# anuragranj/cc

Hardware: AMD Instinct MI355X
Metric: train images/sec (832x256, 5-frame sample, 6-scale CC step) (higher is better)
Workload: dtype f32; 1 GPU; full CC: DispResNet6+PoseNetB6+MaskNet6+Back2Future, all losses; per_gpu_batch=4, global_batch=4, height=256, width=832, scales=6, frames=5, parallelism=dp1, hipgraph=True, trained_nets=all, rccl_ranks=1, dead_occlusion_decoders_elided=False, net_streams=2, pipeline=per_network, grad_chunks=False, deterministic=True

## Files before the change

cc_amd/build.py:

```python
import glob
import os
import subprocess
import sys
from concurrent.futures import ThreadPoolExecutor

HERE = os.path.dirname(os.path.abspath(__file__))
CSRC = os.path.join(HERE, "csrc")
OUT = os.path.join(HERE, "libccengine.so")
OBJ = os.path.join(HERE, "csrc", "_obj")
HIPCC = os.environ.get("HIPCC", "/opt/rocm/bin/hipcc")
FLAGS = ["--offload-arch=gfx950", "-O3", "-std=c++17", "-fPIC", "-ffp-contract=off",
         "-Wno-unused-result", "-I", os.path.join(os.path.dirname(HERE), "include")]


FILE_FLAGS = {"ssim.hip": ["-fno-slp-vectorize"]}


def sources():
    return sorted(glob.glob(os.path.join(CSRC, "*.hip")))


def _stale(target, deps):
    if not os.path.exists(target):
        return True
    t = os.path.getmtime(target)
    return any(os.path.getmtime(d) > t for d in deps)


def source_hash():
    import hashlib
    h = hashlib.sha1()
    files = sorted(glob.glob(os.path.join(CSRC, "*.hip")) + glob.glob(os.path.join(CSRC, "*.h")) +
                   glob.glob(os.path.join(os.path.dirname(HERE), "include", "*.h")))
    for f in files:
        h.update(os.path.basename(f).encode())
        h.update(open(f, "rb").read())
    return int(h.hexdigest()[:8], 16)


TOOLS_OUT = os.path.join(os.path.dirname(HERE), "tools", "_bin", "libccengine_tools.so")


def build_tools(verbose=False, force=False):
    return build(verbose, force, out=TOOLS_OUT, obj=os.path.join(CSRC, "_obj_tools"), extra=["-DCC_TOOLS"])


def build(verbose=False, force=False, out=None, obj=None, extra=()):
    OUT_, OBJ_ = out or OUT, obj or OBJ
# ... 42 lines not shown
```

cc_amd/config.py:

```python
align_corners = False

strict_nan_checks = False

deterministic = True

net_streams = True


grad_chunks = False

bias_table = False

loss_stream = True


class _Debug:
    no_slice_gy = False
    no_wgrad_defer = False
    no_sum_n = False
    no_wgrad_list = False
    no_wgrad_queue = False
    force_comm = False
    capture_mode = "thread_local"
    net_stream_priority = (0, 0, 0)
    chunk_inline = False
    pipe_extra = {}
    pipe_skip_tail = ()
    reduce_trace = None
    library_path = None


debug = _Debug()
```

cc_amd/csrc/corr.hip:

```cpp
#include "cc_common.h"
#include "../../include/ccengine.h"

namespace {

constexpr int R = 4, PATCH = 9, ND = 81;

__global__ __launch_bounds__(256) void k_corr_fwd(const float* __restrict__ f1, const float* __restrict__ f2,
                                                  float* __restrict__ out, const int* __restrict__ chan_of_disp, int C,
                                                  int H, int W, int out_cstride_total, int out_coffset) {
    const int HW = H * W;
    const int p = blockIdx.x * 256 + threadIdx.x;
    const int dy = blockIdx.y, b = blockIdx.z;
    if (p >= HW) return;
    const int y = p / W, x = p - y * W;
    const int yy = y + dy - R;
    float acc[PATCH];
#pragma unroll
    for (int j = 0; j < PATCH; j++) acc[j] = 0.f;
    if (yy >= 0 && yy < H) {
        const float* a = f1 + (size_t)b * C * HW + p;
        const float* bb = f2 + (size_t)b * C * HW + yy * W;
        for (int c = 0; c < C; c++) {
            const float av = a[(size_t)c * HW];
            const float* row = bb + (size_t)c * HW;
// ... 290 lines not shown
    out[((size_t)b * ND2 + d) * HW + p] = acc / (float)C;
}

__global__ __launch_bounds__(256) void k_corrp_bwd(const float* __restrict__ gout, const float* __restrict__ f1,
                                                   const float* __restrict__ f2, float* __restrict__ g1, float* __restrict__ g2,
                                                   int C, int H, int W, int P, int D) {
    const int HW = H * W, ND2 = P * P, r = (P - 1) / 2;
    const int p = blockIdx.x * 256 + threadIdx.x;
    const int c = blockIdx.y, b = blockIdx.z;
    if (p >= HW) return;
    const int y = p / W, x = p - y * W;
    const float* g = gout + (size_t)b * ND2 * HW;
    const float* s1 = f1 + ((size_t)b * C + c) * HW;
    const float* s2 = f2 + ((size_t)b * C + c) * HW;
    float a1 = 0.f, a2 = 0.f;
    for (int i = 0; i < P; i++) {
        const int dy = (i - r) * D;
        for (int j = 0; j < P; j++) {
            const int dx = (j - r) * D, d = i * P + j;
            const int yy = y + dy, xx = x + dx;
            if (yy >= 0 && yy < H && xx >= 0 && xx < W) a1 = fmaf(g[(size_t)d * HW + p], s2[yy * W + xx], a1);
            const int ys = y - dy, xs = x - dx;
            if (ys >= 0 && ys < H && xs >= 0 && xs < W) {
                const int q = ys * W + xs;
                a2 = fmaf(g[(size_t)d * HW + q], s1[q], a2);
            }
        }
    }
    const size_t o = ((size_t)b * C + c) * HW + p;
    if (g1) g1[o] = a1 / (float)C;
    if (g2) g2[o] = a2 / (float)C;
}

}

extern "C" {

int cc_corr9x9_fwd(const float* f1, const float* f2, float* out, const int* chan_of_disp_or_null, int B, int C, int H,
                   int W, int out_channels_total, int out_channel_offset, void* stream) {
    if (B <= 0 || C <= 0 || H <= 0 || W <= 0 || out_channel_offset + ND > out_channels_total) return CC_ERR_ARG;
    const bool v4 = (W % 4 == 0) && (((uintptr_t)f1 | (uintptr_t)f2 | (uintptr_t)out) % 16 == 0);
    if (v4)
        hipLaunchKernelGGL(k_corr_fwd4, dim3((H * (W / 4) + 255) / 256, PATCH, B), dim3(256), 0, (hipStream_t)stream, f1, f2, out,
                           chan_of_disp_or_null, C, H, W, out_channels_total, out_channel_offset);
    else if (H * W <= 4096)
        hipLaunchKernelGGL(k_corr_fwd_small, dim3((H * W * ND + 255) / 256, B), dim3(256), 0, (hipStream_t)stream, f1, f2, out,
                           chan_of_disp_or_null, C, H, W, out_channels_total, out_channel_offset);
    else
        hipLaunchKernelGGL(k_corr_fwd, dim3((H * W + 255) / 256, PATCH, B), dim3(256), 0, (hipStream_t)stream, f1, f2, out,
                           chan_of_disp_or_null, C, H, W, out_channels_total, out_channel_offset);
    CC_CHECK_LAUNCH();
    return CC_OK;
}

int cc_corr9x9_bwd(const float* gout, const float* f1, const float* f2, float* g1, float* g2_or_null,
                   const int* chan_of_disp_or_null, int B, int C, int H, int W, int g_channels_total,
                   int g_channel_offset, int accumulate_g1, void* stream) {
    if (B <= 0 || C <= 0 || H <= 0 || W <= 0 || g_channel_offset + ND > g_channels_total) return CC_ERR_ARG;
    hipStream_t s = (hipStream_t)stream;
    const bool v4 = (W % 4 == 0) &&
                    (((uintptr_t)gout | (uintptr_t)f1 | (uintptr_t)f2 | (uintptr_t)g1 | (uintptr_t)g2_or_null) % 16 == 0);
    if (v4) {
        dim3 g4((H * (W / 4) + 255) / 256, (C + 3) / 4, B);
        hipLaunchKernelGGL(k_corr_bwd_f1_4, g4, dim3(256), 0, s, gout, f2, g1, chan_of_disp_or_null, C, H, W, g_channels_total,
                           g_channel_offset, accumulate_g1);
        if (g2_or_null)
            hipLaunchKernelGGL(k_corr_bwd_f2_4, g4, dim3(256), 0, s, gout, f1, g2_or_null, chan_of_disp_or_null, C, H, W,
                               g_channels_total, g_channel_offset);
        CC_CHECK_LAUNCH();
        return CC_OK;
    }
    dim3 g((H * W + 255) / 256, C, B);
    hipLaunchKernelGGL(k_corr_bwd_f1, g, dim3(256), 0, s, gout, f2, g1, chan_of_disp_or_null, C, H, W, g_channels_total,
                       g_channel_offset, accumulate_g1);
    if (g2_or_null)
        hipLaunchKernelGGL(k_corr_bwd_f2, g, dim3(256), 0, s, gout, f1, g2_or_null, chan_of_disp_or_null, C, H, W,
                           g_channels_total, g_channel_offset);
    CC_CHECK_LAUNCH();
    return CC_OK;
}

int cc_corr_patch_fwd(const float* f1, const float* f2, float* out, int B, int C, int H, int W, int patch, int dilation,
                      void* stream) {
    if (B <= 0 || C <= 0 || H <= 0 || W <= 0 || patch < 1 || (patch & 1) == 0 || dilation < 1) return CC_ERR_ARG;
    const long n = (long)H * W * patch * patch;
    hipLaunchKernelGGL(k_corrp_fwd, dim3((unsigned)((n + 255) / 256), B), dim3(256), 0, (hipStream_t)stream, f1, f2, out, C, H, W,
                       patch, dilation);
    CC_CHECK_LAUNCH();
    return CC_OK;
}

int cc_corr_patch_bwd(const float* gout, const float* f1, const float* f2, float* g1_or_null, float* g2_or_null, int B, int C,
                      int H, int W, int patch, int dilation, void* stream) {
    if (B <= 0 || C <= 0 || H <= 0 || W <= 0 || patch < 1 || (patch & 1) == 0 || dilation < 1) return CC_ERR_ARG;
    hipLaunchKernelGGL(k_corrp_bwd, dim3((H * W + 255) / 256, C, B), dim3(256), 0, (hipStream_t)stream, gout, f1, f2, g1_or_null,
                       g2_or_null, C, H, W, patch, dilation);
    CC_CHECK_LAUNCH();
    return CC_OK;
}

}
```

cc_amd/models/back2future.py:

```python
import torch
import torch.nn as nn
import torch.nn.functional as F

from .. import config
from .. import nn as L
from .. import ops
from ..inverse_warp import feature_warp
from ..tape import run_network


def conv_feat_block(nIn, nOut):
    return nn.Sequential(L.Conv2d(nIn, nOut, 3, 2, 1, act="lrelu"), L.Act(),
                         L.Conv2d(nOut, nOut, 3, 1, 1, act="lrelu"), L.Act())


def conv_dec_block(nIn):
    chans = [nIn, 128, 128, 96, 64, 32]
    layers = []
    for a, b in zip(chans[:-1], chans[1:]):
        layers += [L.Conv2d(a, b, 3, 1, 1, act="lrelu"), L.Act()]
    layers.append(L.Conv2d(32, 2, 3, 1, 1))
    return nn.Sequential(*layers)


# ... 55 lines not shown
                out = tape.conv_group([xs[k] for k in idx], [convs[k].weight for k in idx], [convs[k].bias for k in idx], 1, 1, act)
                for k, y in zip(idx, out):
                    ys[k] = y
            xs = ys
        return xs

    def _body(self, tape, n0, n1, n2):
        ac = config.align_corners
        feats = {}
        xs = [n0, n2, n1]
        for lvl in range(1, 7):
            blocks = [getattr(self, "conv%d%s" % (lvl, s)) for s in "abc"]
            ys = tape.conv_group(xs, [b[0].weight for b in blocks], [b[0].bias for b in blocks], 2, 1, "lrelu")
            xs = tape.conv_group(ys, [b[2].weight for b in blocks], [b[2].bias for b in blocks], 1, 1, "lrelu")
            for s, x in zip("abc", xs):
                feats[(lvl, s)] = x
        flow_f, flow_b, up_f, up_b, occ_raw = {}, {}, {}, {}, {}
        bw, cw = feats[(6, "b")], feats[(6, "c")]
        inv_b, inv_c = ops._inv_perm(self.idx_fwd, n0.t.device), ops._inv_perm(self.idx_bwd, n0.t.device)
        for lvl in range(6, 1, -1):
            a = feats[(lvl, "a")]
            B, C, H, W = a.t.shape
            if lvl == 6:
                cb_o = tape.concat(B, [162, C], H, W, a.t) if not self.elide_occ else None
                corr = tape.corr_pair(a, bw, cw, inv_b, inv_c, out=cb_o.slot(0) if cb_o is not None else None)
                in_f = in_b = corr
                if cb_o is not None:
                    cb_o.put(0, corr)
                    cb_o.put(1, a)
                    in_o = cb_o.done()
            else:
                cb_f = tape.concat(B, [162, C, 2], H, W, a.t)
                cb_b = tape.concat(B, [162, C, 2], H, W, a.t)
                corr = tape.corr_pair(a, bw, cw, inv_b, inv_c, out=cb_f.slot(0))
                cb_f.put(0, corr)
                cb_f.put(1, a)
                cb_f.put(2, up_f[lvl + 1])
                cb_b.buf[:, :162 + C].copy_(cb_f.buf[:, :162 + C])
                cb_b.parts[0], cb_b.parts[1] = corr, a
                cb_b.put(2, up_b[lvl + 1])
                in_f, in_b = cb_f.done(), cb_b.done()
                in_o = in_f
            decs = [getattr(self, "decoder_fwd%d" % lvl), getattr(self, "decoder_bwd%d" % lvl)]
            ins = [in_f, in_b]
            if not self.elide_occ:
                decs.append(getattr(self, "decoder_occ%d" % lvl))
                ins.append(in_o)
            outs = self._decoders(tape, decs, ins)
            flow_f[lvl], flow_b[lvl] = outs[0], outs[1]
            up_f[lvl] = tape.upsample2x(flow_f[lvl])
            up_b[lvl] = tape.upsample2x(flow_b[lvl])
            if not self.elide_occ:
                occ_raw[lvl] = outs[2]
            if lvl > 2:
                s = self.WARP_SCALE[lvl]
                bw = tape.feature_warp(feats[(lvl - 1, "b")], up_f[lvl], s, ac)
                cw = tape.feature_warp(feats[(lvl - 1, "c")], up_f[lvl], -s, ac)
        ff = [tape.upsample2x(up_f[l], self.FULL_SCALE[l]) for l in range(2, 7)]
        fb = [tape.upsample2x(up_b[l], -self.FULL_SCALE[l]) for l in range(2, 7)]
        if self.training and self.nlevels == 6:
            ff += tape.torch_fn([up_f[6]], lambda t: (0.625 * t,))
            fb += tape.torch_fn([up_b[6]], lambda t: (-0.625 * t,))
        if not self.training:
            ff, fb = ff[:1], fb[:1]
        self._n_flow = len(ff)
        return ff + fb + [occ_raw[l] for l in sorted(occ_raw)]

    def forward(self, im_tar, im_refs):
        n = self.normalize([im_tar] + list(im_refs))
        outs = list(run_network(self._body, n, list(self.parameters())))
        k = self._n_flow
# ... 11 lines not shown
```

cc_amd/ops.py:

```python
import torch
import torch.nn.functional as F

from ._lib import engine, image_dense, STREAM
from .config import debug as _dbg

ACT = {None: 0, "relu": 1, "lrelu": 2, "sigmoid": 3}


def _c(t):
    return t.contiguous().float()


def _slice_or_c(t):
    if (t.dtype == torch.float32 and not t.is_contiguous() and image_dense(t) and t.data_ptr() % 16 == 0 and t.stride(0) % 4 == 0
            and not _dbg.no_slice_gy):
        return t, t.stride(0)
    t = _c(t)
    return t, t.shape[1] * t.shape[2] * t.shape[3]


def _ws(nbytes, ref):
    return torch.empty(max(int(nbytes) // 4, 4), device=ref.device, dtype=torch.float32)


# ... 757 lines not shown
        gy, gy_bs = _slice_or_c(gy)
        gx = torch.empty(B, C, H, W, device=gy.device, dtype=torch.float32)
        engine().call("cc_upsample2x_bwd", gy, gx, B, C, H, W, gy_bs, C * H * W, scale, 0, STREAM)
        return gx, None


def upsample_bilinear2x(x, scale=1.0):
    return _Up2xFn.apply(x, float(scale))


_perm_cache = {}


def _inv_perm(perm, device):
    key = (tuple(perm), str(device))
    t = _perm_cache.get(key)
    if t is None:
        inv = [0] * len(perm)
        for k, d in enumerate(perm):
            inv[d] = k
        t = torch.tensor(inv, dtype=torch.int32, device=device)
        _perm_cache[key] = t
    return t


class _CorrPairFn(torch.autograd.Function):

    @staticmethod
    def forward(ctx, a, b, c, inv_b, inv_c):
        a, b, c = _c(a), _c(b), _c(c)
        B, C, H, W = a.shape
        out = torch.empty(B, 162, H, W, device=a.device, dtype=torch.float32)
        E = engine()
        E.call("cc_corr9x9_fwd", a, b, out, inv_b, B, C, H, W, 162, 0, STREAM)
        E.call("cc_corr9x9_fwd", a, c, out, inv_c, B, C, H, W, 162, 81, STREAM)
        ctx.save_for_backward(a, b, c, inv_b, inv_c)
        return out

    @staticmethod
    def backward(ctx, g):
        a, b, c, inv_b, inv_c = ctx.saved_tensors
        g = _c(g)
        B, C, H, W = a.shape
        E = engine()
        ga = torch.empty_like(a)
        gb = torch.empty_like(b) if ctx.needs_input_grad[1] else None
        gc = torch.empty_like(c) if ctx.needs_input_grad[2] else None
        E.call("cc_corr9x9_bwd", g, a, b, ga, gb, inv_b, B, C, H, W, 162, 0, 0, STREAM)
        E.call("cc_corr9x9_bwd", g, a, c, ga, gc, inv_c, B, C, H, W, 162, 81, 1, STREAM)
        return ga, gb, gc, None, None


def correlation_pair(a, b, c, perm_b, perm_c):
    return _CorrPairFn.apply(a, b, c, _inv_perm(perm_b, a.device), _inv_perm(perm_c, a.device))


def correlate(input1, input2):
    a, b = _c(input1), _c(input2)
    return _CorrFn.apply(a, b)


class _CorrFn(torch.autograd.Function):
    @staticmethod
    def forward(ctx, a, b):
        B, C, H, W = a.shape
        out = torch.empty(B, 81, H, W, device=a.device, dtype=torch.float32)
        engine().call("cc_corr9x9_fwd", a, b, out, None, B, C, H, W, 81, 0, STREAM)
        ctx.save_for_backward(a, b)
        return out

    @staticmethod
    def backward(ctx, g):
        a, b = ctx.saved_tensors
        B, C, H, W = a.shape
        ga, gb = torch.empty_like(a), torch.empty_like(b)
        engine().call("cc_corr9x9_bwd", _c(g), a, b, ga, gb, None, B, C, H, W, 81, 0, 0, STREAM)
        return ga, gb


class _CorrPatchFn(torch.autograd.Function):
    @staticmethod
    def forward(ctx, a, b, patch, dilation):
# ... 21 lines not shown
```

cc_amd/tape.py:

```python
import ctypes

import torch

from . import config, ops
from ._lib import engine, STREAM

ACT = ops.ACT


def _bs(t):
    return t.stride(0)


def _new(shape, ref):
    return torch.empty(shape, device=ref.device, dtype=torch.float32)


def _dense(t):
    B, C, H, W = t.shape
    st = t.stride()
    return st[3] == 1 and st[2] == W and st[1] == H * W and (B == 1 or st[0] >= C * H * W)



# ... 504 lines not shown
            assert not (wg and bg) or acc_w == acc_b

            def write(gx, accumulate):
                dst = gx if not accumulate else torch.empty_like(gx)
                E.call("cc_bn_train_bwd", g, xt, mod.weight, mean, invstd, dst, gw, gb, ops._ws(E.call("cc_bn_ws_bytes", C), xt),
                       B, C, H, W, int(acc_w or acc_b), STREAM)
                if accumulate:
                    gx.add_(dst)
            if x.needs:
                x.from_writer(write)
            else:
                x.skip()
                write(torch.empty_like(xt), False)
        self._node(bwd)
        return yt

    def upsample2x(self, x, scale=1.0, out=None):
        E = self.E
        B, C, H, W = x.t.shape
        y = out if out is not None else _new((B, C, 2 * H, 2 * W), x.t)
        E.call("cc_upsample2x_fwd", x.t, y, B, C, H, W, _bs(x.t), _bs(y), float(scale), STREAM)
        yt = self._tt(y)
        self._use(x)
        if self.record:
            def bwd():
                g, _ = yt.final()
                if g is None:
                    x.skip()
                    return
                x.from_writer(lambda gx, acc: E.call("cc_upsample2x_bwd", g, gx, B, C, H, W, _bs(g), _bs(gx), float(scale), int(acc), STREAM))
            self._node(bwd)
        return yt

    def corr_pair(self, a, b, c, inv_b, inv_c, out=None):
        E = self.E
        B, C, H, W = a.t.shape
        at, bt, ct = [t.t if t.t.is_contiguous() else t.t.contiguous() for t in (a, b, c)]
        if out is None:
            out = _new((B, 162, H, W), at)
        tot = _bs(out) // (H * W)
        E.call("cc_corr9x9_fwd", at, bt, out, inv_b, B, C, H, W, tot, 0, STREAM)
        E.call("cc_corr9x9_fwd", at, ct, out, inv_c, B, C, H, W, tot, 81, STREAM)
        yt = self._tt(out)
        self._use(a, b, c)
        if self.record:
            def bwd():
                g, _ = yt.final()
                if g is None:
                    a.skip(), b.skip(), c.skip()
                    return
                gtot = _bs(g) // (H * W)
                ga, gb_, gc = torch.empty_like(at), torch.empty_like(bt), torch.empty_like(ct)
                E.call("cc_corr9x9_bwd", g, at, bt, ga, gb_ if b.needs else None, inv_b, B, C, H, W, gtot, 0, 0, STREAM)
                E.call("cc_corr9x9_bwd", g, at, ct, ga, gc if c.needs else None, inv_c, B, C, H, W, gtot, 81, 1, STREAM)
                a.add_alias(ga)
                b.add_alias(gb_) if b.needs else b.skip()
                c.add_alias(gc) if c.needs else c.skip()
            self._node(bwd)
        return yt

    def feature_warp(self, x, flow, flow_scale, align_corners):
        E = self.E
        xt = x.t if x.t.is_contiguous() else x.t.contiguous()
        ft = flow.t if flow.t.is_contiguous() else flow.t.contiguous()
        B, C, H, W = xt.shape
        y = torch.empty_like(xt)
        E.call("cc_feature_warp_fwd", xt, ft, y, B, C, H, W, int(align_corners), float(flow_scale), STREAM)
        yt = self._tt(y)
        self._use(x, flow)
        if self.record:
            def bwd():
                g, _ = yt.final()
                if g is None:
                    x.skip(), flow.skip()
                    return
                g = g if g.is_contiguous() else g.contiguous()
                gflow = torch.empty_like(ft) if flow.needs else None
                if x.needs:
                    def write(gx, acc):
                        if config.deterministic and C >= 16:
                            ws = torch.empty(int(E.call("cc_feature_warp_bwd_det_ws_bytes", B, C, H, W)), dtype=torch.uint8,
                                             device=gx.device)
                            E.call("cc_feature_warp_bwd_det", g, xt, ft, gflow, gx, ws, B, C, H, W, int(align_corners),
                                   float(flow_scale), int(acc), STREAM)
                            return
                        if not acc:
                            gx.zero_()
# ... 99 lines not shown
```

include/ccengine.h:

```cpp
#ifndef CCENGINE_H
#define CCENGINE_H
#include <stddef.h>
#ifdef __cplusplus
extern "C" {
#endif

size_t cc_version(void);


int cc_pixel2cam(const float* depth, const float* Kinv, float* cam, int B, int H, int W, void* stream);
int cc_cam2pixel(const float* cam, const float* P, float* grid, int B, int H, int W, int has_rot, int has_tr, int rewrite_oob,
                 void* stream);
int cc_pixel2cam_bwd(const float* g, const float* depth, const float* Kinv, float* gdepth_or_null, float* gKinv12, float* ws_partials,
                     int B, int H, int W, void* stream);
int cc_cam2pixel_bwd(const float* ggrid, const float* cam, const float* P, float* gcam_or_null, float* gP, float* ws_partials, int B,
                     int H, int W, int has_rot, int has_tr, int rewrite_oob, void* stream);

size_t cc_warp_partials_bytes(int B, int H, int W);

int cc_inverse_warp_fwd(const float* img, const float* depth, const float* P, const float* Kinv, float* out,
                        int B, int C, int H, int W, int padding_border, int align_corners, void* stream);

int cc_inverse_warp_bwd(const float* gout, const float* img, const float* depth, const float* P,
                        const float* Kinv, float* gdepth, float* gP, float* gimg_or_null, float* ws_partials,
// ... 51 lines not shown
size_t cc_elem_num_blocks(int n);

int cc_adaptive_avg_pool(const float* in, float* out, int planes, int H, int W, int h, int w, void* stream);
int cc_pyramid_build(const float* level0, float* out_packed, int nlevels, int planes, int H, int W, void* stream);
int cc_pyramid_build_multi(const long* level0_host, const long* out_packed_host, int nimg, int nlevels, int planes, int H, int W,
                           void* stream);

int cc_flow_noocc(const float* flow_bw, const float* flow_fw, float* out, int B, int H, int W, void* stream);
int cc_rigid_noocc(const float* flows4, float* out, int B, int H, int W, void* stream);
int cc_rigid_noocc_fused(const float* depth, const float* P4, const float* Kinv, float* out, int B, int H, int W, void* stream);

int cc_reduce_add(const float* partials, int n, float coef, float* accum, void* stream);

int cc_edge_smooth_fwd_bwd(const float* img, const float* pred, float* gpred_or_null, float* partials, float* loss_accum,
                           float gscale, int B, int C, int H, int W, void* stream);
int cc_smooth2_fwd_bwd(const float* pred, float* gpred_or_null, float* partials, float* loss_accum, float weight,
                       float gscale, int planes, int H, int W, void* stream);
int cc_bce_ones_fwd_bwd(const float* mask, float* gmask_or_null, float* partials, float* loss_accum, float gscale, int n,
                        void* stream);
int cc_consensus_bce_fwd_bwd(const float* exp_mask, const float* census_bwd, const float* census_fwd,
                             const float* target_bwd, const float* target_fwd, float* gmask_or_null, float* partials,
                             float* loss_accum, float thresh, float wbce, float gscale, int B, int H, int W,
                             void* stream);
int cc_sum_strided(int n, const long* src, const long* src_bs, float* out, long out_bs, int B, long chw, int accumulate,
                   void* stream);
int cc_scale_by_scalar(const float* a, const float* scalar_dev, float* out, int n, void* stream);
int cc_scale_acc_jobs(const long* jobs_host, int njobs, const float* scalar_dev, void* stream);

int cc_corr9x9_fwd(const float* f1, const float* f2, float* out, const int* chan_of_disp_or_null, int B, int C, int H,
                   int W, int out_channels_total, int out_channel_offset, void* stream);
int cc_corr9x9_bwd(const float* gout, const float* f1, const float* f2, float* g1, float* g2_or_null,
                   const int* chan_of_disp_or_null, int B, int C, int H, int W, int g_channels_total,
                   int g_channel_offset, int accumulate_g1, void* stream);
int cc_corr_patch_fwd(const float* f1, const float* f2, float* out, int B, int C, int H, int W, int patch, int dilation,
                      void* stream);
int cc_corr_patch_bwd(const float* gout, const float* f1, const float* f2, float* g1_or_null, float* g2_or_null, int B, int C,
                      int H, int W, int patch, int dilation, void* stream);

size_t cc_conv2d_fwd_ws_bytes(int B, int Cin, int IH, int IW, int Cout, int R, int S, int stride, int pad, int OH, int OW);
int cc_conv2d_fwd(const float* x, const float* w, const float* bias_or_null, const float* res_or_null, float* y, float* ws,
                  const float* prepacked_or_null, int B, int Cin, int IH, int IW, long x_bs, int Cout, int R, int S, int stride,
                  int pad, int OH, int OW, long y_bs, long res_bs, int act, float act_a, float act_b, void* stream);
size_t cc_conv2d_dgrad_ws_bytes(int B, int K, int OH, int OW, int C, int R, int S, int stride, int pad, int IH, int IW);
int cc_conv2d_dgrad(const float* gy, const float* w, const float* bias_or_null, float* gx, float* ws,
                    const float* prepacked_or_null, int B, int K, int OH, int OW, long gy_bs, int C, int R, int S, int stride,
                    int pad, int IH, int IW, long gx_bs, long w_k_stride, long w_c_stride, int act, float act_a, float act_b,
                    void* stream);
size_t cc_conv2d_fwd_pack_floats(int B, int Cin, int IH, int IW, int Cout, int R, int S, int stride, int pad, int OH, int OW);
int cc_conv2d_fwd_pack_desc(int B, int Cin, int IH, int IW, int Cout, int R, int S, int stride, int pad, int OH, int OW,
                            long src_ptr, long pack_base_ptr, long* desc_out_host);
size_t cc_conv2d_dgrad_pack_floats(int B, int K, int OH, int OW, int C, int R, int S, int stride, int pad, int IH, int IW,
                                   long w_k_stride, long w_c_stride);
int cc_conv2d_dgrad_pack_desc(int B, int K, int OH, int OW, int C, int R, int S, int stride, int pad, int IH, int IW,
                              long w_k_stride, long w_c_stride, long src_ptr, long pack_base_ptr, long* desc_out_host);
int cc_repack_table(const long* table_dev, int ndesc, long total_blocks, void* stream);
size_t cc_conv2d_wgrad_ws_bytes(int B, int M, int AH, int AW, int Cin, int R, int S, int si);
int cc_conv2d_wgrad(const float* a, const float* x, float* gw, float* ws, int B, int M, int AH, int AW, long a_bs, int Cin,
                    int IH, int IW, long x_bs, int R, int S, int si, int pad, long o_sm, long o_sc, int accumulate,
                    void* stream);
size_t cc_conv2d_fwd_group_ws_bytes(int G, int B, int Cin, int IH, int IW, int Cout, int R, int S, int stride, int pad, int OH,
                                    int OW);
int cc_conv2d_fwd_group(int G, const long* x, const long* w, const long* bias, const long* res, const long* y, float* ws,
                        const long* prepacked, int B, int Cin, int IH, int IW, long x_bs, int Cout, int R, int S, int stride,
                        int pad, int OH, int OW, long y_bs, long res_bs, int act, float act_a, float act_b, void* stream);
size_t cc_conv2d_dgrad_group_ws_bytes(int G, int B, int K, int OH, int OW, int C, int R, int S, int stride, int pad, int IH, int IW);
int cc_conv2d_dgrad_group(int G, const long* gy, const long* w, const long* bias, const long* gx, const long* mul, float* ws,
// ... 172 lines not shown
```

Before: 250.3 images/s.

## Fuse paired 9x9 correlation forward and backward into single tiled kernels

Adds fused pair kernels that compute both correlation volumes (a·b and a·c) in one launch. The forward kernel stages channel chunks of a, b and c in shared memory with register prefetch, and can also write a second output copy, so Back2Future no longer copies the correlation channels between the forward and backward input buffers. The backward kernel computes ga, gb and gc together and tiles the gradient planes in shared memory. The aim is fewer launches, one read of a shared by both volumes, and less copy traffic, at the cost of much more complex kernels that keep a debug fallback.

New measurement: 250.0 images/s. About the same (-0.1%).

```diff
diff --git a/cc_amd/build.py b/cc_amd/build.py
--- a/cc_amd/build.py
+++ b/cc_amd/build.py
@@ -13,7 +13,7 @@
          "-Wno-unused-result", "-I", os.path.join(os.path.dirname(HERE), "include")]
 
 
-FILE_FLAGS = {"ssim.hip": ["-fno-slp-vectorize"]}
+FILE_FLAGS = {"ssim.hip": ["-fno-slp-vectorize"], "corr.hip": ["-fno-slp-vectorize"]}
 
 
 def sources():
diff --git a/cc_amd/config.py b/cc_amd/config.py
--- a/cc_amd/config.py
+++ b/cc_amd/config.py
@@ -20,6 +20,7 @@
     no_sum_n = False
     no_wgrad_list = False
     no_wgrad_queue = False
+    no_corr_pair = False
     force_comm = False
     capture_mode = "thread_local"
     net_stream_priority = (0, 0, 0)
diff --git a/cc_amd/csrc/corr.hip b/cc_amd/csrc/corr.hip
--- a/cc_amd/csrc/corr.hip
+++ b/cc_amd/csrc/corr.hip
@@ -346,6 +346,467 @@
     if (g2) g2[o] = a2 / (float)C;
 }
 
+template <int EW>
+__device__ __forceinline__ void pair_ldg(const float* __restrict__ p, bool ok, float (&v)[EW]) {
+    if constexpr (EW == 4) {
+        const float4 t = *(const float4*)p;
+        v[0] = ok ? t.x : 0.f; v[1] = ok ? t.y : 0.f; v[2] = ok ? t.z : 0.f; v[3] = ok ? t.w : 0.f;
+    } else {
+        const float t = *p;
+        v[0] = ok ? t : 0.f;
+    }
+}
+template <int EW>
+__device__ __forceinline__ void pair_sts(float* p, const float (&v)[EW]) {
+    if constexpr (EW == 4) *(float4*)p = make_float4(v[0], v[1], v[2], v[3]);
+    else *p = v[0];
+}
+
+template <int PXW, int NV, int CK, bool VEC>
+__global__ __launch_bounds__(192 * 2 / NV, PXW == 4 && NV == 1 ? 4 : 3) void k_corr_pair_fwd(const float* __restrict__ fa, const float* __restrict__ fb,
+                                                       const float* __restrict__ fc, float* __restrict__ out,
+                                                       float* __restrict__ out2, const int* __restrict__ chan_b,
+                                                       const int* __restrict__ chan_c, int C, int H, int W, int tot, int tot2,
+                                                       int tiles_x) {
+    constexpr int TW = PXW == 4 ? 32 : 16, TH = PXW == 4 ? 8 : 4, NDY = 3, NT = 64 * NDY * 2 / NV;
+    constexpr int HR = TH + NDY - 1, HWP = TW + 8, QPR = TW / PXW, EW = VEC ? 4 : 1;
+    constexpr int NA = CK * TH * TW / EW, NB = CK * HR * HWP / EW, SA = (NA + NT - 1) / NT, SB = (NB + NT - 1) / NT;
+    static_assert(QPR * TH == 64 && (NV == 1 || NV == 2), "one wave per dy (and volume)");
+    __shared__ float4 sA4[CK * TH * TW / 4], sB4[CK * HR * HWP / 4], sC4[CK * HR * HWP / 4];
+    float* sA = (float*)sA4;
+    float* sB = (float*)sB4;
+    float* sC = (float*)sC4;
+    const int tid = threadIdx.x, wv = tid >> 6, lane = tid & 63, r = lane / QPR, q = lane - r * QPR;
+    const int dyl = NV == 2 ? wv : wv >> 1, vol0 = NV == 2 ? 0 : wv & 1;
+    const float* sW0 = vol0 ? sC : sB;
+    const int ty = blockIdx.x / tiles_x, tx = blockIdx.x - ty * tiles_x;
+    const int x0 = tx * TW, y0 = ty * TH, dy0 = blockIdx.y * NDY, bz = blockIdx.z, HW = H * W;
+    const float* pa = fa + (size_t)bz * C * HW;
+    const float* pb = fb + (size_t)bz * C * HW;
+    const float* pc = fc + (size_t)bz * C * HW;
+    int oa[SA], ob[SB];
+#pragma unroll
+    for (int i = 0; i < SA; i++) {
+        const int e = i * NT + tid;
+        oa[i] = -1;
+        if (e < NA) {
+            const int k = e / (TH * TW / EW), rem = e - k * (TH * TW / EW), rr = rem / (TW / EW);
+            const int y = y0 + rr, x = x0 + (rem - rr * (TW / EW)) * EW;
+            if (y < H && x < W) oa[i] = k * HW + y * W + x;
+        }
+    }
+#pragma unroll
+    for (int i = 0; i < SB; i++) {
+        const int e = i * NT + tid;
+        ob[i] = -1;
+        if (e < NB) {
+            const int k = e / (HR * HWP / EW), rem = e - k * (HR * HWP / EW), rr = rem / (HWP / EW);
+            const int y = y0 + dy0 - R + rr, x = x0 - R + (rem - rr * (HWP / EW)) * EW;
+            if (y >= 0 && y < H && x >= 0 && x < W) ob[i] = k * HW + y * W + x;
+        }
+    }
+    float ra[SA][EW], rb[SB][EW], rc[SB][EW];
+    auto fetch = [&](int c0) {
+        const unsigned lim = (unsigned)((C - c0 < CK ? C - c0 : CK) * HW);
+        const size_t base = (size_t)c0 * HW;
+#pragma unroll
+        for (int i = 0; i < SA; i++) {
+            const bool ok = (unsigned)oa[i] < lim;
+            pair_ldg<EW>(pa + base + (ok ? oa[i] : 0), ok, ra[i]);
+        }
+#pragma unroll
+        for (int i = 0; i < SB; i++) {
+            const bool ok = (unsigned)ob[i] < lim;
+            pair_ldg<EW>(pb + base + (ok ? ob[i] : 0), ok, rb[i]);
+            pair_ldg<EW>(pc + base + (ok ? ob[i] : 0), ok, rc[i]);
+        }
+    };
+    auto commit = [&]() {
+#pragma unroll
+        for (int i = 0; i < SA; i++) {
+            const int e = i * NT + tid;
+            if (e < NA) pair_sts<EW>(sA + e * EW, ra[i]);
+        }
+#pragma unroll
+        for (int i = 0; i < SB; i++) {
+            const int e = i * NT + tid;
+            if (e < NB) {
+                pair_sts<EW>(sB + e * EW, rb[i]);
+                pair_sts<EW>(sC + e * EW, rc[i]);
+            }
+        }
+    };
+    float acc[NV][PATCH][PXW];
+#pragma unroll
+    for (int v = 0; v < NV; v++)
+#pragma unroll
+        for (int j = 0; j < PATCH; j++)
+#pragma unroll
+            for (int k = 0; k < PXW; k++) acc[v][j][k] = 0.f;
+    auto channel = [&](int k) {
+        float av[PXW], vw[NV][PXW + 8];
+        const int ia = (k * TH + r) * TW + q * PXW, iw = (k * HR + r + dyl) * HWP + q * PXW;
+        if constexpr (PXW == 4) {
+            const float4 t = *(const float4*)(sA + ia);
+            av[0] = t.x; av[1] = t.y; av[2] = t.z; av[3] = t.w;
+        } else {
+            av[0] = sA[ia];
+        }
+#pragma unroll
+        for (int v = 0; v < NV; v++) {
+            const float* sW = NV == 2 ? (v ? sC : sB) : sW0;
+            if constexpr (PXW == 4) {
+#pragma unroll
+                for (int m = 0; m < 3; m++) {
+                    const float4 u = *(const float4*)(sW + iw + 4 * m);
+                    vw[v][4 * m] = u.x; vw[v][4 * m + 1] = u.y; vw[v][4 * m + 2] = u.z; vw[v][4 * m + 3] = u.w;
+                }
+            } else {
+#pragma unroll
+                for (int m = 0; m < PATCH; m++) vw[v][m] = sW[iw + m];
+            }
+        }
+#pragma unroll
+        for (int v = 0; v < NV; v++)
+#pragma unroll
+            for (int j = 0; j < PATCH; j++)
+#pragma unroll
+                for (int p = 0; p < PXW; p++) acc[v][j][p] = fmaf(av[p], vw[v][p + j], acc[v][j][p]);
+    };
+    fetch(0);
+    commit();
+    __syncthreads();
+    for (int c0 = 0; c0 < C; c0 += CK) {
+        const bool more = c0 + CK < C;
+        if (more) fetch(c0 + CK);
+        const int kmax = C - c0;
+#pragma unroll
+        for (int k = 0; k < CK; k++) {
+            if (k < kmax) channel(k);
+            if constexpr (PXW == 4 && NV == 2) __builtin_amdgcn_sched_barrier(0);
+        }
+        __syncthreads();
+        if (more) commit();
+        __syncthreads();
+    }
+    const int y = y0 + r, x = x0 + q * PXW, dy = dy0 + dyl;
+    if (y >= H || x >= W) return;
+    const float inv = 1.f / (float)C;
+#pragma unroll
+    for (int v = 0; v < NV; v++) {
+        const int vol = NV == 2 ? v : vol0;
+        const int* tab = vol ? chan_c : chan_b;
+#pragma unroll
+        for (int j = 0; j < PATCH; j++) {
+            const int d = dy * PATCH + j;
+            const int ch = (tab ? tab[d] : d) + vol * ND;
+            const size_t o = ((size_t)bz * tot + ch) * HW + y * W + x, o2 = ((size_t)bz * tot2 + ch) * HW + y * W + x;
+            if constexpr (VEC && PXW == 4) {
+                const float4 t = make_float4(acc[v][j][0] * inv, acc[v][j][1] * inv, acc[v][j][2] * inv, acc[v][j][3] * inv);
+                *(float4*)(out + o) = t;
+                if (out2) *(float4*)(out2 + o2) = t;
+            } else {
+#pragma unroll
+                for (int p = 0; p < PXW; p++) {
+                    if (x + p >= W) break;
+                    const float t = acc[v][j][p] * inv;
+                    out[o + p] = t;
+                    if (out2) out2[o2 + p] = t;
+                }
+            }
+        }
+    }
+}
+
+template <bool VEC, bool SIDE>
+__global__ __launch_bounds__(256, SIDE ? 2 : 3) void k_corr_pair_bwd(const float* __restrict__ gout, const float* __restrict__ fa,
+                                                       const float* __restrict__ fb, const float* __restrict__ fc,
+                                                       float* __restrict__ ga, float* __restrict__ gb, float* __restrict__ gc,
+                                                       const int* __restrict__ chan_b, const int* __restrict__ chan_c, int C, int H,
+                                                       int W, int gtot, int tiles_x) {
+    constexpr int TW = 16, TH = 8, HWP = TW + 8, NT = 256, CPT = 2, EW = VEC ? 4 : 1;
+    constexpr int N1 = 18 * TH * TW / EW, N2 = 18 * TH * HWP / EW, S1 = (N1 + NT - 1) / NT, S2 = (N2 + NT - 1) / NT;
+    __shared__ float4 sG1v[18 * TH * TW / 4], sG2v[18 * TH * HWP / 4];
+    __shared__ int sCh[2 * ND];
+    float* sG1 = (float*)sG1v;
+    float* sG2 = (float*)sG2v;
+    const int tid = threadIdx.x, q = tid & 3, r = (tid >> 2) & 7, cg = tid >> 5;
+    const int ty = blockIdx.x / tiles_x, tx = blockIdx.x - ty * tiles_x;
+    const int x0 = tx * TW, y0 = ty * TH, bz = blockIdx.z, HW = H * W;
+    const int y = y0 + r, x = x0 + 4 * q, c0 = blockIdx.y * (8 * CPT) + cg * CPT;
+    for (int i = tid; i < 2 * ND; i += NT) {
+        const int* tab = i < ND ? chan_b : chan_c;
+        const int d = i < ND ? i : i - ND;
+        sCh[i] = (tab ? tab[d] : d) + (i < ND ? 0 : ND);
+    }
+    __syncthreads();
+    const float* g = gout + (size_t)bz * gtot * HW;
+    const float* pa = fa + (size_t)bz * C * HW;
+    const float* pb = fb + (size_t)bz * C * HW;
+    const float* pc = fc + (size_t)bz * C * HW;
+    float rb[CPT][4], rc[CPT][4], sb[CPT][4], sc[CPT][4];
+#pragma unroll
+    for (int cc = 0; cc < CPT; cc++)
+#pragma unroll
+        for (int k = 0; k < 4; k++) rb[cc][k] = rc[cc][k] = sb[cc][k] = sc[cc][k] = 0.f;
+    auto window = [&](const float* __restrict__ img, unsigned row, bool rowok, float (&v)[12]) {
+        if constexpr (VEC) {
+#pragma unroll
+            for (int m = 0; m < 3; m++) {
+                const int xx = x - 4 + 4 * m;
+                const bool ok = rowok && xx >= 0 && xx < W;
+                float4 t = make_float4(0.f, 0.f, 0.f, 0.f);
+                if (ok) t = *(const float4*)(img + (row + (unsigned)xx));
+                v[4 * m] = t.x; v[4 * m + 1] = t.y; v[4 * m + 2] = t.z; v[4 * m + 3] = t.w;
+            }
+        } else {
+#pragma unroll
+            for (int m = 0; m < 12; m++) {
+                const int xx = x - 4 + m;
+                const bool ok = rowok && xx >= 0 && xx < W;
+                v[m] = ok ? img[row + (unsigned)xx] : 0.f;
+            }
+        }
+    };
+#pragma unroll 1
+    for (int dy = 0; dy < PATCH; dy++) {
+        const int yy = y + dy - R, ys = y - dy + R;
+        const bool yyok = yy >= 0 && yy < H, ysok = ys >= 0 && ys < H;
+        float s1[S1][EW], s2[S2][EW];
+#pragma unroll
+        for (int i = 0; i < S1; i++) {
+            const int e = i * NT + tid;
+            bool ok = false;
+            unsigned o = 0;
+            if (e < N1) {
+                const int j = e / (TH * TW / EW), rem = e - j * (TH * TW / EW), rr = rem / (TW / EW);
+                const int py = y0 + rr, px = x0 + (rem - rr * (TW / EW)) * EW;
+                ok = py < H && px < W;
+                if (ok) o = (unsigned)(sCh[(j / PATCH) * ND + dy * PATCH + j % PATCH] * HW + py * W + px);
+            }
+            pair_ldg<EW>(g + o, ok, s1[i]);
+        }
+#pragma unroll
+        for (int i = 0; i < S2; i++) {
+            const int e = i * NT + tid;
+            bool ok = false;
+            unsigned o = 0;
+            if (SIDE && e < N2) {
+                const int j = e / (TH * HWP / EW), rem = e - j * (TH * HWP / EW), rr = rem / (HWP / EW);
+                const int py = y0 + rr - dy + R, px = x0 - R + (rem - rr * (HWP / EW)) * EW;
+                ok = py >= 0 && py < H && px >= 0 && px < W;
+                if (ok) o = (unsigned)(sCh[(j / PATCH) * ND + dy * PATCH + j % PATCH] * HW + py * W + px);
+            }
+            pair_ldg<EW>(g + o, ok, s2[i]);
+        }
+        __syncthreads();
+#pragma unroll
+        for (int i = 0; i < S1; i++) {
+            const int e = i * NT + tid;
+            if (e < N1) pair_sts<EW>(sG1 + e * EW, s1[i]);
+        }
+        if constexpr (SIDE) {
+#pragma unroll
+            for (int i = 0; i < S2; i++) {
+                const int e = i * NT + tid;
+                if (e < N2) pair_sts<EW>(sG2 + e * EW, s2[i]);
+            }
+        }
+        float wb[CPT][12], wc[CPT][12];
+#pragma unroll
+        for (int cc = 0; cc < CPT; cc++) {
+            const int c = (c0 + cc < C) ? c0 + cc : C - 1;
+            const unsigned row = (unsigned)(c * HW + (yyok ? yy : 0) * W);
+            window(pb, row, yyok, wb[cc]);
+            window(pc, row, yyok, wc[cc]);
+        }
+        __syncthreads();
+#pragma unroll
+        for (int dx = 0; dx < PATCH; dx++) {
+#pragma unroll
+            for (int v = 0; v < 2; v++) {
+                const float4 t = *(const float4*)(sG1 + ((v * PATCH + dx) * TH + r) * TW + 4 * q);
+                const float g4[4] = {t.x, t.y, t.z, t.w};
+#pragma unroll
+                for (int cc = 0; cc < CPT; cc++)
+#pragma unroll
+                    for (int k = 0; k < 4; k++) {
+                        if (v == 0) rb[cc][k] = fmaf(g4[k], wb[cc][k + dx], rb[cc][k]);
+                        else rc[cc][k] = fmaf(g4[k], wc[cc][k + dx], rc[cc][k]);
+                    }
+            }
+            __builtin_amdgcn_sched_barrier(0);
+        }
+        if constexpr (SIDE) {
+            float wa[CPT][12];
+#pragma unroll
+            for (int cc = 0; cc < CPT; cc++) {
+                const int c = (c0 + cc < C) ? c0 + cc : C - 1;
+                window(pa, (unsigned)(c * HW + (ysok ? ys : 0) * W), ysok, wa[cc]);
+            }
+#pragma unroll
+            for (int dx = 0; dx < PATCH; dx++) {
+#pragma unroll
+                for (int v = 0; v < 2; v++) {
+                    float gw[4];
+                    const float* row = sG2 + ((v * PATCH + dx) * TH + r) * HWP + 4 * q + 8 - dx;
+#pragma unroll
+                    for (int k = 0; k < 4; k++) gw[k] = row[k];
+#pragma unroll
+                    for (int cc = 0; cc < CPT; cc++)
+#pragma unroll
+                        for (int k = 0; k < 4; k++) {
+                            if (v == 0) sb[cc][k] = fmaf(gw[k], wa[cc][k + 8 - dx], sb[cc][k]);
+                            else sc[cc][k] = fmaf(gw[k], wa[cc][k + 8 - dx], sc[cc][k]);
+                        }
+                }
+                __builtin_amdgcn_sched_barrier(0);
+            }
+        }
+    }
+    if (y >= H || x >= W) return;
+    const float fC = (float)C;
+#pragma unroll
+    for (int cc = 0; cc < CPT; cc++) {
+        if (c0 + cc >= C) break;
+        const size_t o = ((size_t)bz * C + c0 + cc) * HW + y * W + x;
+        float va[4], vb[4], vc[4];
+#pragma unroll
+        for (int k = 0; k < 4; k++) {
+            va[k] = rb[cc][k] / fC + rc[cc][k] / fC;
+            vb[k] = sb[cc][k] / fC;
+            vc[k] = sc[cc][k] / fC;
+        }
+        if constexpr (VEC) {
+            *(float4*)(ga + o) = make_float4(va[0], va[1], va[2], va[3]);
+            if (gb) *(float4*)(gb + o) = make_float4(vb[0], vb[1], vb[2], vb[3]);
+            if (gc) *(float4*)(gc + o) = make_float4(vc[0], vc[1], vc[2], vc[3]);
+        } else {
+#pragma unroll
+            for (int k = 0; k < 4; k++) {
+                if (x + k >= W) break;
+                ga[o + k] = va[k];
+                if (gb) gb[o + k] = vb[k];
+                if (gc) gc[o + k] = vc[k];
+            }
+        }
+    }
+}
+
+__global__ __launch_bounds__(256) void k_corr_pair_fwd_small(const float* __restrict__ fa, const float* __restrict__ fb,
+                                                             const float* __restrict__ fc, float* __restrict__ out,
+                                                             float* __restrict__ out2, const int* __restrict__ chan_b,
+                                                             const int* __restrict__ chan_c, int C, int H, int W, int tot, int tot2) {
+    const int HW = H * W;
+    const int t = blockIdx.x * 256 + threadIdx.x;
+    const int b = blockIdx.y;
+    if (t >= HW * 2 * ND) return;
+    const int d2 = t / HW, p = t - d2 * HW;
+    const int vol = d2 >= ND, d = d2 - vol * ND;
+    const int dy = d / PATCH, dx = d - dy * PATCH;
+    const int y = p / W, x = p - y * W;
+    const int yy = y + dy - R, xx = x + dx - R;
+    float acc = 0.f;
+    if (yy >= 0 && yy < H && xx >= 0 && xx < W) {
+        const float* a = fa + (size_t)b * C * HW + p;
+        const float* bb = (vol ? fc : fb) + (size_t)b * C * HW + yy * W + xx;
+        int c = 0;
+        for (; c + 8 <= C; c += 8) {
+            float av[8], bv[8];
+#pragma unroll
+            for (int k = 0; k < 8; k++) { av[k] = a[(size_t)(c + k) * HW]; bv[k] = bb[(size_t)(c + k) * HW]; }
+#pragma unroll
+            for (int k = 0; k < 8; k++) acc = fmaf(av[k], bv[k], acc);
+        }
+        for (; c < C; c++) acc = fmaf(a[(size_t)c * HW], bb[(size_t)c * HW], acc);
+    }
+    const int* tab = vol ? chan_c : chan_b;
+    const int ch = (tab ? tab[d] : d) + vol * ND;
+    const float r = acc * (1.f / (float)C);
+    out[((size_t)b * tot + ch) * HW + p] = r;
+    if (out2) out2[((size_t)b * tot2 + ch) * HW + p] = r;
+}
+
+__global__ __launch_bounds__(256) void k_corr_pair_bwd_small(const float* __restrict__ gout, const float* __restrict__ fa,
+                                                             const float* __restrict__ fb, const float* __restrict__ fc,
+                                                             float* __restrict__ ga, float* __restrict__ gb, float* __restrict__ gc,
+                                                             const int* __restrict__ chan_b, const int* __restrict__ chan_c, int C,
+                                                             int H, int W, int gtot) {
+    const int HW = H * W;
+    const int p = blockIdx.x * 256 + threadIdx.x;
+    const int c = blockIdx.y / 3, role = blockIdx.y - 3 * c, b = blockIdx.z;
+    if (p >= HW) return;
+    if ((role == 1 && !gb) || (role == 2 && !gc)) return;
+    const int y = p / W, x = p - y * W;
+    const float* g = gout + (size_t)b * gtot * HW;
+    const size_t o = ((size_t)b * C + c) * HW;
+    if (role == 0) {
+        const float* sb = fb + o;
+        const float* sc = fc + o;
+        float accb = 0.f, accc = 0.f;
+        for (int dy = 0; dy < PATCH; dy++) {
+            const int yy = y + dy - R;
+            if (yy < 0 || yy >= H) continue;
+            float gvb[PATCH], svb[PATCH], gvc[PATCH], svc[PATCH];
+#pragma unroll
+            for (int dx = 0; dx < PATCH; dx++) {
+                const int xx = x + dx - R;
+                const int d = dy * PATCH + dx;
+                const int chb = chan_b ? chan_b[d] : d, chc = (chan_c ? chan_c[d] : d) + ND;
+                const bool in = (xx >= 0) && (xx < W);
+                gvb[dx] = in ? g[(size_t)chb * HW + p] : 0.f;
+                svb[dx] = in ? sb[yy * W + xx] : 0.f;
+                gvc[dx] = in ? g[(size_t)chc * HW + p] : 0.f;
+                svc[dx] = in ? sc[yy * W + xx] : 0.f;
+            }
+#pragma unroll
+            for (int dx = 0; dx < PATCH; dx++) {
+                const int xx = x + dx - R;
+                if (xx >= 0 && xx < W) {
+                    accb = fmaf(gvb[dx], svb[dx], accb);
+                    accc = fmaf(gvc[dx], svc[dx], accc);
+                }
+            }
+        }
+        ga[o + p] = accb / (float)C + accc / (float)C;
+        return;
+    }
+    const int* tab = role == 1 ? chan_b : chan_c;
+    const int coff = role == 1 ? 0 : ND;
+    const float* src = fa + o;
+    float acc = 0.f;
+    for (int dy = 0; dy < PATCH; dy++) {
+        const int ys = y - dy + R;
+        if (ys < 0 || ys >= H) continue;
+        float gv[PATCH], sv[PATCH];
+#pragma unroll
+        for (int dx = 0; dx < PATCH; dx++) {
+            const int xs = x - dx + R;
+            const int d = dy * PATCH + dx;
+            const int ch = (tab ? tab[d] : d) + coff;
+            const bool in = (xs >= 0) && (xs < W);
+            const int q = ys * W + xs;
+            gv[dx] = in ? g[(size_t)ch * HW + q] : 0.f;
+            sv[dx] = in ? src[q] : 0.f;
+        }
+#pragma unroll
+        for (int dx = 0; dx < PATCH; dx++) {
+            const int xs = x - dx + R;
+            if (xs >= 0 && xs < W) acc = fmaf(gv[dx], sv[dx], acc);
+        }
+    }
+    (role == 1 ? gb : gc)[o + p] = acc / (float)C;
+}
+
+template <int PXW, int NV, int CK, bool VEC>
+void launch_pair_fwd(hipStream_t s, const float* a, const float* b, const float* c, float* out, float* out2, const int* chan_b,
+                     const int* chan_c, int B, int C, int H, int W, int tot, int tot2) {
+    constexpr int TW = PXW == 4 ? 32 : 16, TH = PXW == 4 ? 8 : 4;
+    const int tiles_x = (W + TW - 1) / TW, tiles_y = (H + TH - 1) / TH;
+    hipLaunchKernelGGL(HIP_KERNEL_NAME(k_corr_pair_fwd<PXW, NV, CK, VEC>), dim3(tiles_x * tiles_y, 3, B), dim3(192 * 2 / NV), 0, s, a, b, c, out,
+                       out2, chan_b, chan_c, C, H, W, tot, tot2, tiles_x);
+}
+
 }
 
 extern "C" {
@@ -394,6 +855,68 @@
     return CC_OK;
 }
 
+int cc_corr9x9_pair_fwd(const float* a, const float* b, const float* c, float* out, float* out2_or_null,
+                        const int* chan_b_or_null, const int* chan_c_or_null, int B, int C, int H, int W, int out_channels_total,
+                        int out2_channels_total, int variant, void* stream) {
+    if (B <= 0 || C <= 0 || H <= 0 || W <= 0 || 2 * ND > out_channels_total || (out2_or_null && 2 * ND > out2_channels_total) ||
+        variant < 0 || variant > 4 || (long)H * W >= (1L << 27))
+        return CC_ERR_ARG;
+    hipStream_t s = (hipStream_t)stream;
+    const bool v4 = (W % 4 == 0) &&
+                    (((uintptr_t)a | (uintptr_t)b | (uintptr_t)c | (uintptr_t)out | (uintptr_t)out2_or_null) % 16 == 0);
+    const long waves4 = (long)((W + 31) / 32) * ((H + 7) / 8) * B * PATCH;
+    const int form = variant ? variant : (long)H * W <= 512 ? 4 : waves4 >= 2000 ? 1 : waves4 >= 512 ? 3 : 2;
+#define CC_PAIR_FWD(PXW, NV, CKV, CKS)                                                                                          \
+    do {                                                                                                                        \
+        if (v4) launch_pair_fwd<PXW, NV, CKV, true>(s, a, b, c, out, out2_or_null, chan_b_or_null, chan_c_or_null, B, C, H, W,  \
+                                                    out_channels_total, out2_channels_total);                                   \
+        else launch_pair_fwd<PXW, NV, CKS, false>(s, a, b, c, out, out2_or_null, chan_b_or_null, chan_c_or_null, B, C, H, W,     \
+                                                  out_channels_total, out2_channels_total);                                     \
+    } while (0)
+    if (form == 1) CC_PAIR_FWD(4, 2, 4, 2);
+    else if (form == 3) CC_PAIR_FWD(4, 1, 8, 4);
+    else if (form == 2) CC_PAIR_FWD(1, 2, 8, 8);
+    else
+        hipLaunchKernelGGL(k_corr_pair_fwd_small, dim3((H * W * 2 * ND + 255) / 256, B), dim3(256), 0, s, a, b, c, out, out2_or_null,
+                           chan_b_or_null, chan_c_or_null, C, H, W, out_channels_total, out2_channels_total);
+#undef CC_PAIR_FWD
+    CC_CHECK_LAUNCH();
+    return CC_OK;
+}
+
+int cc_corr9x9_pair_bwd(const float* gout, const float* a, const float* b, const float* c, float* ga, float* gb_or_null,
+                        float* gc_or_null, const int* chan_b_or_null, const int* chan_c_or_null, int B, int C, int H, int W,
+                        int g_channels_total, int variant, void* stream) {
+    if (B <= 0 || C <= 0 || H <= 0 || W <= 0 || 2 * ND > g_channels_total || variant < 0 || variant > 2) return CC_ERR_ARG;
+    if ((long)(C > g_channels_total ? C : g_channels_total) * H * W >= (1L << 30)) return CC_ERR_ARG;
+    hipStream_t s = (hipStream_t)stream;
+    const bool v4 = (W % 4 == 0) && (((uintptr_t)gout | (uintptr_t)a | (uintptr_t)b | (uintptr_t)c | (uintptr_t)ga |
+                                      (uintptr_t)gb_or_null | (uintptr_t)gc_or_null) % 16 == 0);
+    const int tiles_x = (W + 15) / 16, tiles_y = (H + 7) / 8;
+    const dim3 grid(tiles_x * tiles_y, (C + 15) / 16, B);
+    if (variant == 2 || (variant == 0 && (long)H * W <= 512)) {
+        if (3L * C > 65535) return CC_ERR_ARG;
+        hipLaunchKernelGGL(k_corr_pair_bwd_small, dim3((H * W + 255) / 256, 3 * C, B), dim3(256), 0, s, gout, a, b, c, ga, gb_or_null,
+                           gc_or_null, chan_b_or_null, chan_c_or_null, C, H, W, g_channels_total);
+        CC_CHECK_LAUNCH();
+        return CC_OK;
+    }
+    const bool side = gb_or_null || gc_or_null;
+#define CC_PAIR_BWD(VEC, SIDE)                                                                                                  \
+    hipLaunchKernelGGL(HIP_KERNEL_NAME(k_corr_pair_bwd<VEC, SIDE>), grid, dim3(256), 0, s, gout, a, b, c, ga, gb_or_null,        \
+                       gc_or_null, chan_b_or_null, chan_c_or_null, C, H, W, g_channels_total, tiles_x)
+    if (v4) {
+        if (side) CC_PAIR_BWD(true, true);
+        else CC_PAIR_BWD(true, false);
+    } else {
+        if (side) CC_PAIR_BWD(false, true);
+        else CC_PAIR_BWD(false, false);
+    }
+#undef CC_PAIR_BWD
+    CC_CHECK_LAUNCH();
+    return CC_OK;
+}
+
 int cc_corr_patch_fwd(const float* f1, const float* f2, float* out, int B, int C, int H, int W, int patch, int dilation,
                       void* stream) {
     if (B <= 0 || C <= 0 || H <= 0 || W <= 0 || patch < 1 || (patch & 1) == 0 || dilation < 1) return CC_ERR_ARG;
diff --git a/cc_amd/models/back2future.py b/cc_amd/models/back2future.py
--- a/cc_amd/models/back2future.py
+++ b/cc_amd/models/back2future.py
@@ -111,11 +111,15 @@
             else:
                 cb_f = tape.concat(B, [162, C, 2], H, W, a.t)
                 cb_b = tape.concat(B, [162, C, 2], H, W, a.t)
-                corr = tape.corr_pair(a, bw, cw, inv_b, inv_c, out=cb_f.slot(0))
+                pair = not config.debug.no_corr_pair
+                corr = tape.corr_pair(a, bw, cw, inv_b, inv_c, out=cb_f.slot(0), out2=cb_b.slot(0) if pair else None)
                 cb_f.put(0, corr)
                 cb_f.put(1, a)
                 cb_f.put(2, up_f[lvl + 1])
-                cb_b.buf[:, :162 + C].copy_(cb_f.buf[:, :162 + C])
+                if pair:
+                    cb_b.buf[:, 162:162 + C].copy_(cb_f.buf[:, 162:162 + C])
+                else:
+                    cb_b.buf[:, :162 + C].copy_(cb_f.buf[:, :162 + C])
                 cb_b.parts[0], cb_b.parts[1] = corr, a
                 cb_b.put(2, up_b[lvl + 1])
                 in_f, in_b = cb_f.done(), cb_b.done()
diff --git a/cc_amd/ops.py b/cc_amd/ops.py
--- a/cc_amd/ops.py
+++ b/cc_amd/ops.py
@@ -813,8 +813,11 @@
         B, C, H, W = a.shape
         out = torch.empty(B, 162, H, W, device=a.device, dtype=torch.float32)
         E = engine()
-        E.call("cc_corr9x9_fwd", a, b, out, inv_b, B, C, H, W, 162, 0, STREAM)
-        E.call("cc_corr9x9_fwd", a, c, out, inv_c, B, C, H, W, 162, 81, STREAM)
+        if _dbg.no_corr_pair:
+            E.call("cc_corr9x9_fwd", a, b, out, inv_b, B, C, H, W, 162, 0, STREAM)
+            E.call("cc_corr9x9_fwd", a, c, out, inv_c, B, C, H, W, 162, 81, STREAM)
+        else:
+            E.call("cc_corr9x9_pair_fwd", a, b, c, out, None, inv_b, inv_c, B, C, H, W, 162, 0, 0, STREAM)
         ctx.save_for_backward(a, b, c, inv_b, inv_c)
         return out
 
@@ -827,8 +830,11 @@
         ga = torch.empty_like(a)
         gb = torch.empty_like(b) if ctx.needs_input_grad[1] else None
         gc = torch.empty_like(c) if ctx.needs_input_grad[2] else None
-        E.call("cc_corr9x9_bwd", g, a, b, ga, gb, inv_b, B, C, H, W, 162, 0, 0, STREAM)
-        E.call("cc_corr9x9_bwd", g, a, c, ga, gc, inv_c, B, C, H, W, 162, 81, 1, STREAM)
+        if _dbg.no_corr_pair:
+            E.call("cc_corr9x9_bwd", g, a, b, ga, gb, inv_b, B, C, H, W, 162, 0, 0, STREAM)
+            E.call("cc_corr9x9_bwd", g, a, c, ga, gc, inv_c, B, C, H, W, 162, 81, 1, STREAM)
+        else:
+            E.call("cc_corr9x9_pair_bwd", g, a, b, c, ga, gb, gc, inv_b, inv_c, B, C, H, W, 162, 0, STREAM)
         return ga, gb, gc, None, None
 
 
diff --git a/cc_amd/tape.py b/cc_amd/tape.py
--- a/cc_amd/tape.py
+++ b/cc_amd/tape.py
@@ -560,15 +560,22 @@
             self._node(bwd)
         return yt
 
-    def corr_pair(self, a, b, c, inv_b, inv_c, out=None):
+    def corr_pair(self, a, b, c, inv_b, inv_c, out=None, out2=None):
         E = self.E
         B, C, H, W = a.t.shape
         at, bt, ct = [t.t if t.t.is_contiguous() else t.t.contiguous() for t in (a, b, c)]
         if out is None:
             out = _new((B, 162, H, W), at)
         tot = _bs(out) // (H * W)
-        E.call("cc_corr9x9_fwd", at, bt, out, inv_b, B, C, H, W, tot, 0, STREAM)
-        E.call("cc_corr9x9_fwd", at, ct, out, inv_c, B, C, H, W, tot, 81, STREAM)
+        pair = not config.debug.no_corr_pair
+        if pair:
+            E.call("cc_corr9x9_pair_fwd", at, bt, ct, out, out2, inv_b, inv_c, B, C, H, W, tot,
+                   _bs(out2) // (H * W) if out2 is not None else 0, 0, STREAM)
+        else:
+            E.call("cc_corr9x9_fwd", at, bt, out, inv_b, B, C, H, W, tot, 0, STREAM)
+            E.call("cc_corr9x9_fwd", at, ct, out, inv_c, B, C, H, W, tot, 81, STREAM)
+            if out2 is not None:
+                out2.copy_(out)
         yt = self._tt(out)
         self._use(a, b, c)
         if self.record:
@@ -579,8 +586,12 @@
                     return
                 gtot = _bs(g) // (H * W)
                 ga, gb_, gc = torch.empty_like(at), torch.empty_like(bt), torch.empty_like(ct)
-                E.call("cc_corr9x9_bwd", g, at, bt, ga, gb_ if b.needs else None, inv_b, B, C, H, W, gtot, 0, 0, STREAM)
-                E.call("cc_corr9x9_bwd", g, at, ct, ga, gc if c.needs else None, inv_c, B, C, H, W, gtot, 81, 1, STREAM)
+                if pair:
+                    E.call("cc_corr9x9_pair_bwd", g, at, bt, ct, ga, gb_ if b.needs else None, gc if c.needs else None, inv_b, inv_c,
+                           B, C, H, W, gtot, 0, STREAM)
+                else:
+                    E.call("cc_corr9x9_bwd", g, at, bt, ga, gb_ if b.needs else None, inv_b, B, C, H, W, gtot, 0, 0, STREAM)
+                    E.call("cc_corr9x9_bwd", g, at, ct, ga, gc if c.needs else None, inv_c, B, C, H, W, gtot, 81, 1, STREAM)
                 a.add_alias(ga)
                 b.add_alias(gb_) if b.needs else b.skip()
                 c.add_alias(gc) if c.needs else c.skip()
diff --git a/include/ccengine.h b/include/ccengine.h
--- a/include/ccengine.h
+++ b/include/ccengine.h
@@ -107,6 +107,12 @@
 int cc_corr9x9_bwd(const float* gout, const float* f1, const float* f2, float* g1, float* g2_or_null,
                    const int* chan_of_disp_or_null, int B, int C, int H, int W, int g_channels_total,
                    int g_channel_offset, int accumulate_g1, void* stream);
+int cc_corr9x9_pair_fwd(const float* a, const float* b, const float* c, float* out, float* out2_or_null,
+                        const int* chan_b_or_null, const int* chan_c_or_null, int B, int C, int H, int W, int out_channels_total,
+                        int out2_channels_total, int variant, void* stream);
+int cc_corr9x9_pair_bwd(const float* gout, const float* a, const float* b, const float* c, float* ga, float* gb_or_null,
+                        float* gc_or_null, const int* chan_b_or_null, const int* chan_c_or_null, int B, int C, int H, int W,
+                        int g_channels_total, int variant, void* stream);
 int cc_corr_patch_fwd(const float* f1, const float* f2, float* out, int B, int C, int H, int W, int patch, int dilation,
                       void* stream);
 int cc_corr_patch_bwd(const float* gout, const float* f1, const float* f2, float* g1_or_null, float* g2_or_null, int B, int C,
```
